# gauravchak/two_tower_models

Measured on AMD Instinct MI355X. Metric: user-item pairs/sec (in-batch softmax train step: fwd + zero_grad + bwd + dense-exact Adam), higher is better.
Workload: dtype f32

## Files before the change

### include/tt_hotpath.h

```cpp
#ifndef TT_HOTPATH_H
#define TT_HOTPATH_H

#include <stdint.h>

#ifdef __cplusplus
extern "C" {
#endif

#define TT_ABI_VERSION 5

#define TT_E_BADARG (-1)
#define TT_E_WORKSPACE (-2)
#define TT_E_UNSUPPORTED (-3)

typedef void* tt_stream_t;

int tt_abi_version(void);
const char* tt_last_error_string(void);

int tt_profile_enable(int on);
int tt_profile_read(const char* kernel, double* total_ms, int64_t* launches);
int tt_profile_filter(const char* kernels);
int tt_profile_pause(int paused);

int tt_gather_rows(const float* table, int64_t n_rows, int64_t dim, const int64_t* ids,
                   int64_t n_ids, float* out, int64_t ld_out, int32_t* oob_flag,
                   tt_stream_t stream);

#define TT_GEMM_NT 0
#define TT_GEMM_NN 1
#define TT_GEMM_TN 2
#define TT_EPI_NONE 0
#define TT_EPI_RELU 1
#define TT_EPI_RELU_MASK 2
int64_t tt_gemm_workspace_bytes(int layout, int64_t M, int64_t N, int64_t K);
int tt_gemm_f32(int layout, int64_t M, int64_t N, int64_t K, const float* A, int64_t lda,
                const float* B, int64_t ldb, float* C, int64_t ldc, const float* bias,
                int epilogue, const float* aux, int64_t ldaux, int accumulate, void* ws,
                int64_t ws_bytes, tt_stream_t stream);
int tt_gemm_tn_colsum_f32(int64_t M, int64_t N, int64_t K, const float* A, int64_t lda, const float* B,
                          int64_t ldb, float* C, int64_t ldc, int accumulate, float* a_colsum, void* ws,
                          int64_t ws_bytes, tt_stream_t stream);
// ... 151 lines not shown
                         const tt_grad_sources* src , int64_t n_ids, const int32_t* sorted_ids,
                         const int32_t* perm, const int32_t* seg_begin, const int32_t* n_unique,
                         void* side, int64_t side_bytes, tt_stream_t stream);

typedef struct {
  const float *W, *M, *V;
  int64_t n_rows, dim;
  const int64_t* ids;
  int64_t n_ids;
  void* side;
  int64_t side_bytes;
} tt_adam_stash_job;
typedef struct {
  float *W, *M, *V;
  int64_t n_rows, dim;
  const tt_grad_sources* src;
  int64_t n_ids;
  const int32_t *sorted_ids, *perm, *seg_begin, *n_unique;
  void* side;
  int64_t side_bytes;
} tt_adam_finish_job;
int tt_adam_begin_ids(double* hyper, float* tab, int64_t tab_steps, const tt_adam_stash_job* jobs, int32_t n_jobs,
                      tt_stream_t stream);
int tt_adam_tables_finish(const tt_adam_finish_job* jobs, int32_t n_jobs, const double* hyper, tt_stream_t stream);
int tt_adam_begin_ids_planes(double* hyper, float* tab, int64_t tab_steps, const tt_adam_stash_job* jobs, int32_t n_jobs,
                             int32_t planes, tt_stream_t stream);

int tt_stream_create_low_priority(void** out_stream);
int tt_stream_destroy(void* stream);

int tt_adam_advance_tab(double* hyper, float* tab, int64_t tab_steps, tt_stream_t stream);
int tt_adam_rows_catchup(float* W, float* M, float* V, int64_t n_rows, int64_t dim, const int64_t* ids,
                         int64_t n_ids, int32_t* last_step, const double* hyper, const float* tab,
                         int64_t tab_steps, tt_stream_t stream);
int tt_adam_table_lazy(float* W, float* M, float* V, int64_t n_rows, int64_t dim, const double* hyper,
                       const tt_grad_sources* src , int64_t n_ids, const int32_t* sorted_ids,
                       const int32_t* perm, const int32_t* seg_begin, const int32_t* n_unique, void* ws,
                       int64_t ws_bytes, int32_t* last_step, const float* tab, int64_t tab_steps,
                       tt_stream_t stream);
int tt_adam_table_flush(float* W, float* M, float* V, int64_t n_rows, int64_t dim, int32_t* last_step,
                        const double* hyper, const float* tab, int64_t tab_steps, tt_stream_t stream);

typedef struct tt_adam_tensor_s {
  float* p;
  const float* g;
  float* m;
  float* v;
  int64_t n;
} tt_adam_tensor;
int tt_adam_dense(const tt_adam_tensor* tensors , int32_t n_tensors, const double* hyper,
                  tt_stream_t stream);
int tt_pack_grads(const tt_adam_tensor* tensors , int32_t n_tensors, tt_stream_t stream);
int tt_copy_buffers(const tt_adam_tensor* buffers , int32_t n_buffers, tt_stream_t stream);
int tt_stream_copy(const void* src, void* dst, int64_t bytes, tt_stream_t stream);
int64_t tt_mfma_probe_flops(int dtype, int32_t iters);
int tt_mfma_probe(int dtype, int32_t iters, float* sink , int64_t sink_floats, tt_stream_t stream);

int tt_hist_embed_pool(const float* table, int64_t n_rows, int64_t dim, const int64_t* ids,
                       int64_t B, int64_t H, const float* pe, float* x, float* pooled,
                       int64_t ld_pooled, int32_t* oob_flag, tt_stream_t stream);
int tt_hist_dx_pool_bwd(const float* dqkv, const float* w_in, int64_t B, int64_t H, int64_t D, const float* d_pooled,
                        int64_t ld_pooled, float* dx, tt_stream_t stream);

int tt_hist_pool_bwd(float* dx, int64_t B, int64_t H, int64_t dim, const float* d_pooled,
                     int64_t ld_pooled, tt_stream_t stream);
int tt_attn_fwd(const float* qkv, int64_t B, int64_t H, int64_t D, int64_t heads, float* ctx,
                float* lse, tt_stream_t stream);
int tt_attn_bwd(const float* qkv, const float* ctx, const float* lse, const float* d_ctx,
                int64_t B, int64_t H, int64_t D, int64_t heads, float* d_qkv, tt_stream_t stream);
int tt_enc_last_supported(int64_t H, int64_t D, int64_t heads);
int tt_enc_last_fwd(const float* x, int64_t B, int64_t H, int64_t D, int64_t heads, const float* w_in,
                    const float* b_in, const float* w_out, const float* b_out, float* recent, int64_t ld_recent,
                    float* q0, float* t, float* probs, float* xbar, float* ctx0, tt_stream_t stream);
int64_t tt_enc_last_bwd_workspace_bytes(int64_t B, int64_t H, int64_t D, int64_t heads);
// ... 109 lines not shown
```

### two_tower_models_amd/_native.py

```python
from __future__ import annotations

import ctypes as C
import os
from typing import Optional

import torch

_PKG = os.path.dirname(os.path.abspath(__file__))
LIB_PATH = os.path.join(_PKG, "lib", "libtt_hotpath.so")

TT_GEMM_NT, TT_GEMM_NN, TT_GEMM_TN = 0, 1, 2
TT_EPI_NONE, TT_EPI_RELU, TT_EPI_RELU_MASK = 0, 1, 2
TT_F32, TT_BF16, TT_F16X2 = 0, 1, 2
TT_E_BADARG, TT_E_WORKSPACE, TT_E_UNSUPPORTED = -1, -2, -3
TT_DEBIAS_COMBINED, TT_DEBIAS_POSITION, TT_DEBIAS_USER = 0, 1, 2
TT_COMM_ID_BYTES = 128
TT_COMM_F32, TT_COMM_I32, TT_COMM_I64, TT_COMM_U8 = 0, 1, 2, 3
TT_COMM_SUM, TT_COMM_MAX = 0, 1
TT_MAX_GRAD_SOURCES = 4
ABI_VERSION = 5

_vp, _i64, _i32, _int = C.c_void_p, C.c_int64, C.c_int32, C.c_int


class GradSources(C.Structure):

    _fields_ = [
        ("rows", _vp * TT_MAX_GRAD_SOURCES),
        ("ld", _i64 * TT_MAX_GRAD_SOURCES),
        ("first", _i64 * (TT_MAX_GRAD_SOURCES + 1)),
        ("n_sources", _i32),
    ]


class AdamTensor(C.Structure):

    _fields_ = [("p", _vp), ("g", _vp), ("m", _vp), ("v", _vp), ("n", _i64)]


class AdamStashJob(C.Structure):

    _fields_ = [("W", _vp), ("M", _vp), ("V", _vp), ("n_rows", _i64), ("dim", _i64), ("ids", _vp), ("n_ids", _i64),
                ("side", _vp), ("side_bytes", _i64)]


class AdamFinishJob(C.Structure):

    _fields_ = [("W", _vp), ("M", _vp), ("V", _vp), ("n_rows", _i64), ("dim", _i64), ("src", C.POINTER(GradSources)),
                ("n_ids", _i64), ("sorted_ids", _vp), ("perm", _vp), ("seg_begin", _vp), ("n_unique", _vp), ("side", _vp),
                ("side_bytes", _i64)]


class TowerFwdSide(C.Structure):
# ... 73 lines not shown
    "tt_inbatch_ce_bwd_kept": (_int, [_vp, _i64, _i64, _i64, _i64, _i64, _vp, _vp, _vp, _i64, _vp, _i64, _vp, _i64, _vp]),
    "tt_ce16_supported": (_int, [_i64, _i64, _i64]),
    "tt_ce16_workspace_bytes": (_i64, [_i64, _i64, _i64]),
    "tt_ce16_fwd_du_keep": (_int, [_vp, _i64, _vp, _i64, _i64, _i64, _i64, _i64, _vp, _vp, _vp, _i64, _vp, _i64, _vp, _i64, _vp]),
    "tt_ce16_bwd_kept": (_int, [_vp, _i64, _i64, _i64, _i64, _i64, _vp, _vp, _vp, _i64, _vp, _i64, _vp, _i64, _vp]),
    "tt_ce16_bwd_recompute": (_int, [_vp, _i64, _vp, _i64, _i64, _i64, _i64, _i64, _vp, _vp, _vp, _i64, _vp, _i64, _int, _vp]),
    "tt_scale_rows": (_int, [_vp, _i64, _vp, _i64, _i64, _vp, _i64, _vp]),
    "tt_weighted_mean_loss": (_int, [_vp, _i64, _i64, _vp, _vp, _vp, _vp, _vp, _vp]),
    "tt_value_weights": (_int, [_vp, _i64, _i64, _vp, _vp, _vp, _vp]),
    "tt_weighted_loss_global": (_int, [_vp, _vp, _vp, _i64, C.c_float, _vp, _vp, _vp]),
    "tt_debias_loss_workspace_bytes": (_i64, [_i64, _i64, _i64]),
    "tt_debias_loss_fwd": (_int, [_int, _vp, _vp, _i64, _i64, _vp, _vp, _i64, _vp, _vp, _i64, _i64, _vp, _vp, _vp, _vp, _i64,
                                  _vp, _vp]),
    "tt_debias_loss_bwd": (_int, [_int, _vp, _vp, _i64, _vp, _i64, _vp, _i64, _i64, _vp, _vp, _i64, _vp, _vp, _i64, _vp, _vp,
                                  _vp, _vp]),
    "tt_rowgrad_workspace_bytes": (_i64, [_i64]),
    "tt_rowgrad_plan": (_int, [_vp, _i64, _i64, _vp, _vp, _vp, _vp, _vp, _vp, _i64, _vp]),
    "tt_rowgrad_dense": (_int, [C.POINTER(GradSources), _i64, _i64, _vp, _vp, _vp, _vp, _vp, _vp]),
    "tt_adam_advance": (_int, [_vp, _vp]),
    "tt_adam_table_workspace_bytes": (_i64, [_i64, _i64]),
    "tt_adam_table": (_int, [_vp, _vp, _vp, _i64, _i64, _vp, C.POINTER(GradSources), _i64, _vp, _vp, _vp,
                             _vp, _vp, _i64, _vp]),
    "tt_adam_table_stash": (_int, [_vp, _vp, _vp, _i64, _i64, _i64, _vp, _vp, _vp, _vp, _vp, _i64, _vp]),
    "tt_adam_table_stash_ids": (_int, [_vp, _vp, _vp, _i64, _i64, _vp, _i64, _vp, _i64, _vp]),
    "tt_adam_table_sweep": (_int, [_vp, _vp, _vp, _i64, _i64, _vp, _vp]),
    "tt_adam_tables_sweep": (_int, [C.POINTER(AdamTensor), _i32, _vp, _i32, _vp]),
    "tt_adam_marks_words": (_i64, [_i64]),
    "tt_adam_marked_supported": (_int, [_i64]),
    "tt_adam_mark_rows": (_int, [_vp, _i64, _i64, _vp, _i64, _vp]),
    "tt_adam_tables_sweep_marked": (_int, [C.POINTER(AdamTensor), C.POINTER(_i64), C.POINTER(_vp), _i32, _vp, _i32, _vp]),
    "tt_adam_table_finish": (_int, [_vp, _vp, _vp, _i64, _i64, _vp, C.POINTER(GradSources), _i64, _vp, _vp, _vp,
                                    _vp, _vp, _i64, _vp]),
    "tt_adam_advance_tab": (_int, [_vp, _vp, _i64, _vp]),
    "tt_adam_rows_catchup": (_int, [_vp, _vp, _vp, _i64, _i64, _vp, _i64, _vp, _vp, _vp, _i64, _vp]),
    "tt_adam_table_lazy": (_int, [_vp, _vp, _vp, _i64, _i64, _vp, C.POINTER(GradSources), _i64, _vp, _vp, _vp, _vp,
                                  _vp, _i64, _vp, _vp, _i64, _vp]),
    "tt_adam_table_flush": (_int, [_vp, _vp, _vp, _i64, _i64, _vp, _vp, _vp, _i64, _vp]),
    "tt_stream_create_low_priority": (_int, [C.POINTER(_vp)]),
    "tt_stream_destroy": (_int, [_vp]),
    "tt_adam_dense": (_int, [C.POINTER(AdamTensor), _i32, _vp, _vp]),
    "tt_pack_grads": (_int, [C.POINTER(AdamTensor), _i32, _vp]),
    "tt_copy_buffers": (_int, [C.POINTER(AdamTensor), _i32, _vp]),
    "tt_hist_embed_pool": (_int, [_vp, _i64, _i64, _vp, _i64, _i64, _vp, _vp, _vp, _i64, _vp, _vp]),
    "tt_hist_dx_pool_bwd": (_int, [_vp, _vp, _i64, _i64, _i64, _vp, _i64, _vp, _vp]),
    "tt_hist_pool_bwd": (_int, [_vp, _i64, _i64, _i64, _vp, _i64, _vp]),
    "tt_attn_fwd": (_int, [_vp, _i64, _i64, _i64, _i64, _vp, _vp, _vp]),
    "tt_attn_bwd": (_int, [_vp, _vp, _vp, _vp, _i64, _i64, _i64, _i64, _vp, _vp]),
    "tt_enc_last_supported": (_int, [_i64, _i64, _i64]),
    "tt_enc_last_fwd": (_int, [_vp, _i64, _i64, _i64, _i64, _vp, _vp, _vp, _vp, _vp, _i64, _vp, _vp, _vp, _vp, _vp, _vp]),
    "tt_enc_last_bwd_workspace_bytes": (_i64, [_i64, _i64, _i64, _i64]),
    "tt_enc_last_bwd": (_int, [_vp, _i64, _i64, _i64, _i64, _vp, _vp, _vp, _i64, _vp, _vp, _vp, _vp, _vp, _vp, _vp, _vp,
                               _vp, _vp, _vp, _i64, _vp]),
    "tt_enc_last_bwd_data": (_int, [_vp, _i64, _i64, _i64, _i64, _vp, _vp, _vp, _i64, _vp, _vp, _vp, _vp, _i64, _vp]),
    "tt_enc_last_bwd_weights": (_int, [_vp, _i64, _i64, _i64, _i64, _vp, _i64, _vp, _vp, _vp, _vp, _vp, _vp, _vp, _vp, _i64, _vp]),
    "tt_stream_copy": (_int, [_vp, _vp, _i64, _vp]),
    "tt_mfma_probe_flops": (_i64, [_int, _i32]),
    "tt_mfma_probe": (_int, [_int, _i32, _vp, _i64, _vp]),
    "tt_rowgrad_plan_jobs_supported": (_int, [_i64]),
    "tt_rowgrad_plan_jobs": (_int, [C.POINTER(PlanJob), _i32, _vp, _vp]),
    "tt_route_workspace_bytes": (_i64, [_i64, _i32]),
    "tt_route_count": (_int, [_vp, _i64, _i64, _i64, _i32, _vp, _vp, _vp, _vp, _i64, _vp]),
    "tt_route_build": (_int, [_vp, _i64, _i64, _i64, _i32, _i64, _vp, _i64, _vp, _vp, _vp, _vp, _vp]),
    "tt_route_localize": (_int, [_vp, _i64, _i64, _i64, _vp, _vp]),
    "tt_route_count_jobs": (_int, [C.POINTER(RouteJob), _i32, _i32, _vp, _vp]),
    "tt_route_build_jobs": (_int, [C.POINTER(RouteJob), _i32, _i32, _vp, _vp]),
    "tt_route_serve_jobs": (_int, [C.POINTER(RouteServeJob), _i32, _vp]),
    "tt_comm_unique_id": (_int, [_vp]),
    "tt_comm_init": (_int, [_vp, _i32, _i32, C.POINTER(_vp)]),
    "tt_comm_destroy": (_int, [_vp]),
    "tt_comm_size": (_int, [_vp, C.POINTER(_i32), C.POINTER(_i32)]),
# ... 182 lines not shown
```

### two_tower_models_amd/csrc/adam.hip

```cpp
#include <stdlib.h>

#include "common.hpp"

namespace tt {

constexpr int SWEEP_MAX_TABLES_DECL = 4;

constexpr int SWEEP_DEFAULT_PERSIST = 3;

struct AdamConst {
  float one_minus_b1, b2, one_minus_b2, eps, neg_step_size, inv_bc2_sqrt;
};

__device__ __forceinline__ AdamConst load_hyper(const double* __restrict__ h) {
  AdamConst c;
  c.one_minus_b1 = (float)(1.0 - h[1]);
  c.b2 = (float)h[2];
  c.one_minus_b2 = (float)(1.0 - h[2]);
  c.eps = (float)h[3];
  c.neg_step_size = (float)(-h[5]);
  c.inv_bc2_sqrt = (float)(1.0 / h[6]);
  return c;
}

// ... 457 lines not shown
__global__ __launch_bounds__(256) void adam_mark_rows_kernel(const int64_t* __restrict__ ids, int64_t n_ids, int64_t n_rows,
                                                             unsigned* __restrict__ marks) {
  const int64_t i = (int64_t)blockIdx.x * 256 + threadIdx.x;
  if (i >= n_ids) return;
  const int64_t row = ids[i];
  if (row >= 0 && row < n_rows) atomicOr(&marks[row >> 5], 1u << (row & 31));
}

__global__ __launch_bounds__(256) void adam_sweep_scalar_kernel(float* __restrict__ W, float* __restrict__ M,
                                                                float* __restrict__ V, int64_t i0, int64_t n,
                                                                const double* __restrict__ hyper) {
  const AdamConst c = load_hyper(hyper);
  const int64_t stride = (int64_t)gridDim.x * blockDim.x;
  for (int64_t i = i0 + (int64_t)blockIdx.x * blockDim.x + threadIdx.x; i < n; i += stride) {
    float p = W[i], m = M[i], v = V[i];
    adam_elem_zero_grad(p, m, v, c);
    W[i] = p; M[i] = m; V[i] = v;
  }
}

__device__ __forceinline__ void replay_consts(AdamConst& c, const double* __restrict__ h, const float* __restrict__ tab,
                                              int64_t cap, int64_t j) {
  if (j < cap) {
    c.neg_step_size = tab[2 * j];
    c.inv_bc2_sqrt = tab[2 * j + 1];
  } else {
    double h5, h6;
    step_consts_from_doubles(h[0], h[1], h[2], (double)j, h5, h6);
    c.neg_step_size = (float)(-h5);
    c.inv_bc2_sqrt = (float)(1.0 / h6);
  }
}

template <int Q>
__device__ __forceinline__ void replay_row_q(float* __restrict__ W, float* __restrict__ M, float* __restrict__ V,
                                             int64_t row, int64_t dim, int32_t from, int32_t to,
                                             const double* __restrict__ hyper, const float* __restrict__ tab,
                                             int64_t cap, int lane) {
  AdamConst c = load_hyper(hyper);
  for (int64_t d0 = 0; d0 < dim; d0 += 64 * Q) {
    float p[Q], m[Q], v[Q];
    bool live = false;
#pragma unroll
    for (int q = 0; q < Q; ++q) {
      const int64_t d = d0 + lane + 64 * q;
      const int64_t at = row * dim + (d < dim ? d : dim - 1);
      p[q] = W[at]; m[q] = M[at]; v[q] = V[at];
      live = live || (d < dim && (m[q] != 0.f || v[q] != 0.f));
    }
    if (!__any(live)) continue;
    for (int32_t j = from + 1; j <= to; ++j) {
      replay_consts(c, hyper, tab, cap, j);
#pragma unroll
      for (int q = 0; q < Q; ++q) adam_elem_zero_grad(p[q], m[q], v[q], c);
    }
#pragma unroll
    for (int q = 0; q < Q; ++q) {
      const int64_t d = d0 + lane + 64 * q;
      if (d < dim) { W[row * dim + d] = p[q]; M[row * dim + d] = m[q]; V[row * dim + d] = v[q]; }
    }
  }
}
__device__ __forceinline__ void replay_row(float* __restrict__ W, float* __restrict__ M, float* __restrict__ V,
                                           int64_t row, int64_t dim, int32_t from, int32_t to,
                                           const double* __restrict__ hyper, const float* __restrict__ tab,
                                           int64_t cap, int lane) {
  from = __builtin_amdgcn_readfirstlane(from);
  to = __builtin_amdgcn_readfirstlane(to);
  if (dim <= 64) replay_row_q<1>(W, M, V, row, dim, from, to, hyper, tab, cap, lane);
  else if (dim <= 128) replay_row_q<2>(W, M, V, row, dim, from, to, hyper, tab, cap, lane);
  else replay_row_q<4>(W, M, V, row, dim, from, to, hyper, tab, cap, lane);
}

__global__ __launch_bounds__(256) void adam_catchup_ids_kernel(float* __restrict__ W, float* __restrict__ M,
                                                               float* __restrict__ V, int64_t n_rows, int64_t dim,
                                                               const int64_t* __restrict__ ids, int64_t n_ids,
                                                               int32_t* __restrict__ last_step,
                                                               const double* __restrict__ hyper, int offset,
                                                               const float* __restrict__ tab, int64_t cap) {
  const int64_t i = (int64_t)blockIdx.x * 4 + (threadIdx.x >> 6);
  if (i >= n_ids) return;
  const int lane = threadIdx.x & 63;
  const int64_t row = ids[i];
  if (row < 0 || row >= n_rows) return;
  const int32_t target = (int32_t)hyper[4] + offset;
  int32_t prev = 0;
  if (lane == 0) prev = atomicMax(&last_step[row], target);
  prev = __shfl(prev, 0, 64);
  if (prev >= target) return;
  replay_row(W, M, V, row, dim, prev, target, hyper, tab, cap, lane);
}

__global__ __launch_bounds__(256) void adam_catchup_plan_kernel(float* __restrict__ W, float* __restrict__ M,
                                                                float* __restrict__ V, int64_t n_rows, int64_t dim,
                                                                const int32_t* __restrict__ sorted_ids,
                                                                const int32_t* __restrict__ seg_begin,
                                                                const int32_t* __restrict__ n_unique,
                                                                int32_t* __restrict__ last_step,
                                                                const double* __restrict__ hyper, int offset, int mark,
                                                                const float* __restrict__ tab, int64_t cap) {
  const int64_t u = (int64_t)blockIdx.x * 4 + (threadIdx.x >> 6);
  if (u >= *n_unique) return;
  const int lane = threadIdx.x & 63;
  const int64_t row = sorted_ids[seg_begin[u]];
  if (row >= n_rows) return;
  const int32_t target = (int32_t)hyper[4] + offset;
  const int32_t prev = last_step[row];
  if (prev < target) replay_row(W, M, V, row, dim, prev, target, hyper, tab, cap, lane);
  if (lane == 0) last_step[row] = target + mark;
}

__global__ __launch_bounds__(256) void adam_flush_kernel(float* __restrict__ W, float* __restrict__ M,
                                                         float* __restrict__ V, int64_t n_rows, int64_t dim,
                                                         int32_t* __restrict__ last_step,
                                                         const double* __restrict__ hyper,
                                                         const float* __restrict__ tab, int64_t cap) {
  const int lane = threadIdx.x & 63;
  const int32_t target = (int32_t)hyper[4];
  const int64_t stride = (int64_t)gridDim.x * 4;
  for (int64_t row = (int64_t)blockIdx.x * 4 + (threadIdx.x >> 6); row < n_rows; row += stride) {
    const int32_t prev = last_step[row];
    if (prev >= target) continue;
    replay_row(W, M, V, row, dim, prev, target, hyper, tab, cap, lane);
    if (lane == 0) last_step[row] = target;
  }
}

constexpr int ADAM_BATCH = 64;
struct AdamBatch { tt_adam_tensor t[ADAM_BATCH]; };
__global__ __launch_bounds__(256) void adam_dense_kernel(const AdamBatch ts, const double* __restrict__ hyper) {
  const tt_adam_tensor t = ts.t[blockIdx.y];
  const AdamConst c = load_hyper(hyper);
  const int64_t stride = (int64_t)gridDim.x * blockDim.x;
  for (int64_t i = (int64_t)blockIdx.x * blockDim.x + threadIdx.x; i < t.n; i += stride) {
    float p = t.p[i], m = t.m[i], v = t.v[i];
    adam_elem(p, m, v, t.g[i], c);
    t.p[i] = p; t.m[i] = m; t.v[i] = v;
  }
}

__global__ __launch_bounds__(256) void pack_grads_kernel(const AdamBatch ts) {
  const tt_adam_tensor t = ts.t[blockIdx.y];
  const int64_t stride = (int64_t)gridDim.x * blockDim.x;
  for (int64_t i = (int64_t)blockIdx.x * blockDim.x + threadIdx.x; i < t.n; i += stride) t.p[i] = t.g[i];
}

__global__ __launch_bounds__(256) void copy_buffers_kernel(const AdamBatch ts) {
  const tt_adam_tensor t = ts.t[blockIdx.y];
  char* dst = reinterpret_cast<char*>(t.p);
  const char* src = reinterpret_cast<const char*>(t.g);
  const int64_t stride = (int64_t)gridDim.x * blockDim.x, i0 = (int64_t)blockIdx.x * blockDim.x + threadIdx.x;
  const bool vec = ((reinterpret_cast<uintptr_t>(dst) | reinterpret_cast<uintptr_t>(src)) & 15) == 0;
  const int64_t n16 = vec ? t.n / 16 : 0;
  for (int64_t i = i0; i < n16; i += stride) reinterpret_cast<uint4*>(dst)[i] = reinterpret_cast<const uint4*>(src)[i];
  for (int64_t i = n16 * 16 + i0; i < t.n; i += stride) dst[i] = src[i];
}
// ... 337 lines not shown
      if (rc) return rc;
    }
    return 0;
  }
  FinishJobs a{};
  a.n = n_jobs;
  unsigned blocks = 0;
  const int rows_per_block = 256 / lpr;
  for (int i = 0; i < n_jobs; ++i) {
    const tt_adam_finish_job& j = jobs[i];
    a.W[i] = j.W; a.M[i] = j.M; a.V[i] = j.V; a.n_rows[i] = j.n_rows; a.dim[i] = j.dim; a.cap[i] = j.n_ids;
    a.src[i] = *j.src; a.sorted_ids[i] = j.sorted_ids; a.perm[i] = j.perm; a.seg_begin[i] = j.seg_begin; a.n_unique[i] = j.n_unique;
    a.side[i] = reinterpret_cast<const float*>(j.side);
    a.first_block[i] = blocks;
    blocks += (unsigned)ceil_div(j.n_ids, rows_per_block);
  }
  for (int i = n_jobs; i <= SWEEP_MAX_TABLES; ++i) a.first_block[i] = blocks;
  hipStream_t st = S(stream);
  if (lpr == 16) adam_finish_tables_kernel<16><<<blocks, 256, 0, st>>>(a, hyper);
  else if (lpr == 32) adam_finish_tables_kernel<32><<<blocks, 256, 0, st>>>(a, hyper);
  else adam_finish_tables_kernel<64><<<blocks, 256, 0, st>>>(a, hyper);
  return check_launch("adam_finish_tables_kernel");
}

extern "C" int tt_adam_advance_tab(double* hyper, float* tab, int64_t tab_steps, tt_stream_t stream) {
  if (!hyper || !tab) return fail_arg("tt_adam_advance_tab: null pointer");
  if (tab_steps <= 0) return fail_arg("tt_adam_advance_tab: sizes");
  adam_advance_kernel<<<1, 1, 0, S(stream)>>>(hyper, tab, tab_steps);
  return check_launch("adam_advance_kernel");
}

extern "C" int tt_adam_rows_catchup(float* W, float* M, float* V, int64_t n_rows, int64_t dim, const int64_t* ids,
                                    int64_t n_ids, int32_t* last_step, const double* hyper, const float* tab,
                                    int64_t tab_steps, tt_stream_t stream) {
  if (!W || !M || !V || !ids || !last_step || !hyper || !tab) return fail_arg("tt_adam_rows_catchup: null pointer");
  if (n_rows <= 0 || dim <= 0 || n_ids <= 0) return fail_arg("tt_adam_rows_catchup: sizes");
  adam_catchup_ids_kernel<<<(unsigned)ceil_div(n_ids, 4), 256, 0, S(stream)>>>(W, M, V, n_rows, dim, ids, n_ids, last_step, hyper, 0, tab, tab_steps);
  return check_launch("adam_catchup_ids_kernel");
}

extern "C" int tt_adam_table_lazy(float* W, float* M, float* V, int64_t n_rows, int64_t dim, const double* hyper,
                                  const tt_grad_sources* src, int64_t n_ids, const int32_t* sorted_ids,
                                  const int32_t* perm, const int32_t* seg_begin, const int32_t* n_unique,
                                  void* ws, int64_t ws_bytes, int32_t* last_step, const float* tab,
                                  int64_t tab_steps, tt_stream_t stream) {
  if (!W || !M || !V || !hyper || !sorted_ids || !perm || !seg_begin || !n_unique || !ws || !last_step || !tab)
    return fail_arg("tt_adam_table_lazy: null pointer");
  if (n_rows <= 0 || dim <= 0 || n_ids <= 0) return fail_arg("tt_adam_table_lazy: sizes");
  if (!check_sources(src, n_ids, dim)) return fail_arg("tt_adam_table_lazy: gradient sources");
  if (ws_bytes < tt_adam_table_workspace_bytes(n_ids, dim)) { set_error("tt_adam_table_lazy: workspace"); return TT_E_WORKSPACE; }
  hipStream_t st = S(stream);
  const unsigned blocks = (unsigned)ceil_div(n_ids, 4);
  adam_catchup_plan_kernel<<<blocks, 256, 0, st>>>(W, M, V, n_rows, dim, sorted_ids, seg_begin, n_unique, last_step, hyper, -1, 1, tab, tab_steps);
  int rc = check_launch("adam_catchup_plan_kernel");
  if (rc) return rc;
  adam_touched_kernel<false><<<blocks, 256, 0, st>>>(W, M, V, n_rows, dim, hyper, *src, sorted_ids, perm, seg_begin, n_unique, reinterpret_cast<float*>(ws), n_ids);
  if ((rc = check_launch("adam_touched_kernel"))) return rc;
  adam_writeback_kernel<<<blocks, 256, 0, st>>>(W, M, V, n_rows, dim, sorted_ids, seg_begin, perm, n_unique, reinterpret_cast<const float*>(ws), n_ids);
  return check_launch("adam_writeback_kernel");
}

extern "C" int tt_adam_table_flush(float* W, float* M, float* V, int64_t n_rows, int64_t dim, int32_t* last_step,
                                   const double* hyper, const float* tab, int64_t tab_steps, tt_stream_t stream) {
  if (!W || !M || !V || !last_step || !hyper || !tab) return fail_arg("tt_adam_table_flush: null pointer");
  if (n_rows <= 0 || dim <= 0) return fail_arg("tt_adam_table_flush: sizes");
  const int64_t want = ceil_div(n_rows, 4);
  const int64_t cap = (int64_t)device_cu_count() * 32;
  ProfScope prof("adam_flush_kernel", S(stream));
  adam_flush_kernel<<<(unsigned)(want < cap ? want : cap), 256, 0, S(stream)>>>(W, M, V, n_rows, dim, last_step, hyper, tab, tab_steps);
  return check_launch("adam_flush_kernel");
}

extern "C" int tt_adam_dense(const tt_adam_tensor* tensors, int32_t n_tensors, const double* hyper,
                             tt_stream_t stream) {
  if (!tensors || !hyper) return fail_arg("tt_adam_dense: null pointer");
  if (n_tensors <= 0) return fail_arg("tt_adam_dense: sizes");
  for (int32_t base = 0; base < n_tensors; base += ADAM_BATCH) {
    const int32_t cnt = (n_tensors - base < ADAM_BATCH) ? n_tensors - base : ADAM_BATCH;
    AdamBatch b;
    int64_t max_n = 1;
    for (int32_t i = 0; i < cnt; ++i) {
      b.t[i] = tensors[base + i];
      if (!b.t[i].p || !b.t[i].g || !b.t[i].m || !b.t[i].v || b.t[i].n < 0) return fail_arg("tt_adam_dense: descriptor");
      if (b.t[i].n > max_n) max_n = b.t[i].n;
    }
    const int64_t bx = ceil_div(max_n, 1024) < 1024 ? ceil_div(max_n, 1024) : 1024;
    adam_dense_kernel<<<dim3((unsigned)bx, (unsigned)cnt), 256, 0, S(stream)>>>(b, hyper);
    const int rc = check_launch("adam_dense_kernel");
    if (rc) return rc;
  }
  return 0;
}

extern "C" int tt_pack_grads(const tt_adam_tensor* tensors, int32_t n_tensors, tt_stream_t stream) {
  if (!tensors) return fail_arg("tt_pack_grads: null pointer");
  if (n_tensors <= 0) return fail_arg("tt_pack_grads: sizes");
  for (int32_t base = 0; base < n_tensors; base += ADAM_BATCH) {
    const int32_t cnt = (n_tensors - base < ADAM_BATCH) ? n_tensors - base : ADAM_BATCH;
    AdamBatch b;
    int64_t max_n = 1;
    for (int32_t i = 0; i < cnt; ++i) {
      b.t[i] = tensors[base + i];
// ... 70 lines not shown
```

### two_tower_models_amd/optim.py

```python
from __future__ import annotations

import ctypes as C
import os
import sys
import weakref
from typing import Dict, Iterable, List, Optional, Sequence

import torch

from . import _native as N
from . import ops


_RELEASE_AT_LOGITS = True
_SPLIT_MIN_IDS = 65536
_MARK_ROWS = True
_HOLD_SWEEP = True


class _TableStep:

    __slots__ = ("plan", "side", "announced", "marked", "n_rows")

    def __init__(self, plan, side, announced=False, marked=False, n_rows=0):
# ... 20 lines not shown
                 eps: float = 1e-8, overlap_sweep=True, lazy: bool = False) -> None:
        if lr < 0 or eps < 0 or not (0 <= betas[0] < 1) or not (0 <= betas[1] < 1):
            raise ValueError("invalid Adam hyper-parameters")
        super().__init__(params, dict(lr=lr, betas=betas, eps=eps))
        if len(self.param_groups) != 1:
            raise ValueError("DenseExactAdam supports a single parameter group")
        self._params: List[torch.nn.Parameter] = [p for p in self.param_groups[0]["params"]]
        self._tables = [p for p in self._params if getattr(p, "_tt_is_table", False)]
        self._dense = [p for p in self._params if not getattr(p, "_tt_is_table", False)]
        for p in self._tables:
            p._tt_rowgrads = []
            p._tt_lookups = []
            p._tt_active = None
            p._tt_optimizer = weakref.ref(self)
        if overlap_sweep not in (True, False, "forward"):
            raise ValueError('overlap_sweep must be True, False or "forward"')
        self._sharded = [p for p in self._tables if getattr(p, "_tt_shard", None) is not None]
        if self._sharded:
            if len(self._sharded) != len(self._tables):
                raise ValueError("either every embedding table of the model is row-sharded or none is")
            if lazy:
                raise ValueError("the deferred (lazy) schedule is a single-GPU schedule; row-sharded tables use the dense-exact sweep")
            overlap_sweep = "forward"
        self._flat_g: Optional[torch.Tensor] = None
        self.lazy = bool(lazy)
        self.overlap_sweep = False if self.lazy else overlap_sweep
        self._last_step: Dict[int, torch.Tensor] = {}
        self._tab: Optional[torch.Tensor] = None
        self._tab_steps = 0
        self._host_steps = 0
        self._resume_step = 0
        self._prefetch_done: Optional[torch.cuda.Event] = None
        self._prefetch_keep = None
        if self.lazy:
            for p in self._tables:
                p._tt_lazy = _LazyRows(self, p)
        self._hyper = None
        self._ready = False
        self._side_stream: Optional[torch.cuda.Stream] = None
        self.capture_overlap = False
        self._sweep_wgs = 0
        self._tune = None
        self._tune_done: List[list] = []
        self._tune_state = None
        self._plan_stream: Optional[torch.cuda.Stream] = None
        self._plan_done: Optional[torch.cuda.Event] = None
        self._plans_pending = False
        self._plan_ready: Optional[torch.cuda.Event] = None
        self._begun: Optional[Dict[torch.nn.Parameter, _TableStep]] = None
        self._sweep_done: Optional[torch.cuda.Event] = None
        self._side_bufs: Dict[int, torch.Tensor] = {}
        self._marks: Dict[int, torch.Tensor] = {}
        self._sweep_pending = None
        self._sweep_pending_marked = False
        self._sweep_events = None
        self._catchup_last: Dict[int, tuple] = {}

    def _init_state(self) -> None:
        dev = N.require_device(*self._params)
        g = self.param_groups[0]
        self._hyper = torch.tensor([g["lr"], g["betas"][0], g["betas"][1], g["eps"], 0.0, 0.0, 0.0, 0.0],
                                   dtype=torch.float64, device=dev)
        arena = bool(self._tables) and all(p.is_cuda for p in self._tables) and os.environ.get("TT_ADAM_NO_ARENA") is None
        in_arena = {id(p) for p in self._tables} if arena else set()
        for p in self._params:
            if p.dtype != torch.float32 or not p.is_contiguous():
# ... 75 lines not shown
        if rates:
            torch.cuda.empty_cache()
        self.arena_note = {"candidates_GBps": [round(r, 1) for r in rates], "kept": best, "bytes": nbytes}
        with torch.no_grad():
            for p, (home, m, v) in zip(self._tables, views(arena)):
                st = self.state[p]
                home.copy_(p.data)
                p.data = home
                for key, t in (("exp_avg", m), ("exp_avg_sq", v)):
                    if key in st:
                        t.copy_(st[key])
                    else:
                        t.zero_()
                    st[key] = t
        self._arena = arena

    def _catch_up(self, p: torch.nn.Parameter, ids: torch.Tensor) -> None:
        if not self._ready or self._host_steps == 0 or not p.is_cuda or ids.numel() == 0:
            return
        cur = torch.cuda.current_stream()
        if self._prefetch_done is not None:
            cur.wait_event(self._prefetch_done)
        if ops._aux_forks[0]:
            prev = self._catchup_last.get(id(p))
            if prev is not None and prev[1] != cur:
                cur.wait_event(prev[0])
        ids = ids.reshape(-1)
        if ids.dtype != torch.int64 or not ids.is_contiguous():
            ids = ids.to(torch.int64).contiguous()
        st = self.state[p]
        N.check(N.load().tt_adam_rows_catchup(p.data_ptr(), st["exp_avg"].data_ptr(), st["exp_avg_sq"].data_ptr(),
                                              p.shape[0], p.shape[1], ids.data_ptr(), ids.numel(),
                                              self._last_step[id(p)].data_ptr(), self._hyper.data_ptr(),
                                              self._tab.data_ptr(), self._tab_steps, N.stream()),
                "tt_adam_rows_catchup")
        if ops._aux_forks[0]:
            ev = torch.cuda.Event()
            ev.record(cur)
            self._catchup_last[id(p)] = (ev, cur)

    @torch.no_grad()
    def prefetch_rows(self, lookups: Dict[torch.nn.Parameter, Sequence[torch.Tensor]]) -> None:
        if not self.lazy or not self._ready or self._host_steps == 0:
            return
        mine = {id(p): p for p in self._tables}
        main = torch.cuda.current_stream()
        ready = torch.cuda.Event()
        ready.record(main)
        self._side_stream.wait_event(ready)
        lib = N.load()
        keep = []
        for p, blocks in lookups.items():
            if id(p) not in mine or not p.is_cuda:
                continue
            st = self.state[p]
            for ids in blocks:
                ids = ids.reshape(-1)
                if ids.dtype != torch.int64 or not ids.is_contiguous():
                    ids = ids.to(torch.int64).contiguous()
                if ids.numel() == 0:
                    continue
                keep.append(ids)
                N.check(lib.tt_adam_rows_catchup(p.data_ptr(), st["exp_avg"].data_ptr(), st["exp_avg_sq"].data_ptr(),
                                                 p.shape[0], p.shape[1], ids.data_ptr(), ids.numel(),
                                                 self._last_step[id(p)].data_ptr(), self._hyper.data_ptr(),
                                                 self._tab.data_ptr(), self._tab_steps,
                                                 self._side_stream.cuda_stream), "tt_adam_rows_catchup")
        self._prefetch_done = torch.cuda.Event()
        self._prefetch_done.record(self._side_stream)
        self._prefetch_keep = keep

    @torch.no_grad()
    def flush(self) -> None:
        if not self.lazy or not self._ready or self._host_steps == 0:
            return
        if self._prefetch_done is not None:
            torch.cuda.current_stream().wait_event(self._prefetch_done)
            self._prefetch_done, self._prefetch_keep = None, None
        lib = N.load()
        for p in self._tables:
            st = self.state[p]
            N.check(lib.tt_adam_table_flush(p.data_ptr(), st["exp_avg"].data_ptr(), st["exp_avg_sq"].data_ptr(),
                                            p.shape[0], p.shape[1], self._last_step[id(p)].data_ptr(),
                                            self._hyper.data_ptr(), self._tab.data_ptr(), self._tab_steps,
                                            N.stream()), "tt_adam_table_flush")

    def state_dict(self):
        self.flush()
        sd = super().state_dict()
        step = torch.tensor(float(self.step_count))
        for st in sd["state"].values():
            st["step"] = step.clone()
        return sd

    def load_state_dict(self, state_dict) -> None:
        super().load_state_dict(state_dict)
        steps = {int(float(st["step"])) for st in self.state.values() if "step" in st}
        if len(steps) > 1:
            raise ValueError("DenseExactAdam needs one common step count for all parameters")
        self._resume_step = steps.pop() if steps else 0
        self._begun = None
        self._ready = False

    def _advance_lazy(self) -> None:
        if self._host_steps + 2 >= self._tab_steps:
            bigger = torch.zeros(4 * self._tab_steps, dtype=torch.float32, device=self._tab.device)
            bigger[: 2 * self._tab_steps].copy_(self._tab)
            self._tab, self._tab_steps = bigger, 2 * self._tab_steps
        N.check(N.load().tt_adam_advance_tab(self._hyper.data_ptr(), self._tab.data_ptr(), self._tab_steps,
                                             N.stream()), "tt_adam_advance_tab")
        self._host_steps += 1

    @property
    def step_count(self) -> int:
        if not self._ready:
            return int(self._resume_step)
        return int(self._hyper[4].item())

# ... 422 lines not shown
                end = torch.cuda.Event(enable_timing=True)
                end.record()
                self._tune[3] = end
                if len(self._tune_done) < 1024:
                    self._tune_done.append(self._tune)
                self._tune = None
        elif self.lazy:
            if self._prefetch_done is not None:
                torch.cuda.current_stream().wait_event(self._prefetch_done)
                self._prefetch_done, self._prefetch_keep = None, None
            self._catchup_last.clear()
            self._advance_lazy()
            todo = []
            for p in self._tables:
                blocks = p._tt_rowgrads
                if p.grad is not None:
                    raise RuntimeError("embedding table received a dense gradient while in row-gradient mode")
                if not blocks:
                    continue
                if all(b.index is not None for b in blocks):
                    blocks = sorted(blocks, key=lambda b: b.index)
                todo.append((p, blocks, ops.RowPlan([b.ids for b in blocks], p.shape[0], slot=f"plan{len(todo)}", defer=True)))
            ops.RowPlan.build_many([plan for _, _, plan in todo])
            for p, blocks, plan in todo:
                plan.attach([b.rows for b in blocks])
                st = self.state[p]
                n_rows, dim = p.shape
                wsp, wsn = ops._ws(p.device, lib.tt_adam_table_workspace_bytes(plan.n, dim), "adam_side")
                N.check(lib.tt_adam_table_lazy(p.data_ptr(), st["exp_avg"].data_ptr(), st["exp_avg_sq"].data_ptr(),
                                               n_rows, dim, hyper, C.byref(plan.sources), plan.n,
                                               plan.sorted_ids.data_ptr(), plan.perm.data_ptr(),
                                               plan.seg_begin.data_ptr(), plan.n_unique.data_ptr(), wsp, wsn,
                                               self._last_step[id(p)].data_ptr(), self._tab.data_ptr(),
                                               self._tab_steps, N.stream()), "tt_adam_table_lazy")
        else:
            N.check(lib.tt_adam_advance(hyper, N.stream()), "tt_adam_advance")
            self._host_steps += 1
            for p in self._tables:
                blocks = p._tt_rowgrads
                st = self.state[p]
                n_rows, dim = p.shape
                if p.grad is not None:
                    raise RuntimeError("embedding table received a dense gradient while in row-gradient mode")
                if blocks:
                    if all(b.index is not None for b in blocks):
                        blocks = sorted(blocks, key=lambda b: b.index)
                    plan = ops.RowPlan.from_grads(blocks, n_rows)
                    wsp, wsn = ops._ws(p.device, lib.tt_adam_table_workspace_bytes(plan.n, dim), "adam_side")
                    N.check(lib.tt_adam_table(p.data_ptr(), st["exp_avg"].data_ptr(), st["exp_avg_sq"].data_ptr(),
                                              n_rows, dim, hyper, C.byref(plan.sources), plan.n,
                                              plan.sorted_ids.data_ptr(), plan.perm.data_ptr(),
                                              plan.seg_begin.data_ptr(), plan.n_unique.data_ptr(), wsp, wsn,
                                              N.stream()), "tt_adam_table")
        for p in self._tables:
            for b in p._tt_rowgrads:
                b.rows
            p._tt_lookups.clear()
            p._tt_rowgrads.clear()
            p._tt_active = None

        if reduce is not None:
            self._finish_dense_allreduce(reduce, lib, hyper)
            return None
        live = [p for p in self._dense if p.grad is not None]
        if live:
            descs = (N.AdamTensor * len(live))()
            keep = []
# ... 10 lines not shown
```

Baseline: 1.524 million.

## Add frozen-row early exit and float2 packed math to lazy Adam replay

The lazy Adam catch-up replay now runs zero-grad steps in blocks of 16. After each block it checks, wave-wide, whether every parameter has become frozen, meaning the update is too small relative to |p| to change it. Once frozen, it advances only m and v, and stops updating m once it reaches a fixed point. The math is done on packed float2 vectors, and the dim>128 Q=4 path is dropped in favour of Q=2 looping. An environment flag restores the plain per-element replay. This is meant to cut the cost of replaying many skipped steps for rarely touched embedding rows, but it depends on a bit-exactness argument about when p stops changing.

```diff
diff --git a/include/tt_hotpath.h b/include/tt_hotpath.h
--- a/include/tt_hotpath.h
+++ b/include/tt_hotpath.h
@@ -7,7 +7,7 @@
 extern "C" {
 #endif
 
-#define TT_ABI_VERSION 5
+#define TT_ABI_VERSION 6
 
 #define TT_E_BADARG (-1)
 #define TT_E_WORKSPACE (-2)
@@ -225,14 +225,15 @@
 int tt_adam_advance_tab(double* hyper, float* tab, int64_t tab_steps, tt_stream_t stream);
 int tt_adam_rows_catchup(float* W, float* M, float* V, int64_t n_rows, int64_t dim, const int64_t* ids,
                          int64_t n_ids, int32_t* last_step, const double* hyper, const float* tab,
-                         int64_t tab_steps, tt_stream_t stream);
+                         int64_t tab_steps, int32_t replay_plain, tt_stream_t stream);
 int tt_adam_table_lazy(float* W, float* M, float* V, int64_t n_rows, int64_t dim, const double* hyper,
                        const tt_grad_sources* src , int64_t n_ids, const int32_t* sorted_ids,
                        const int32_t* perm, const int32_t* seg_begin, const int32_t* n_unique, void* ws,
                        int64_t ws_bytes, int32_t* last_step, const float* tab, int64_t tab_steps,
-                       tt_stream_t stream);
+                       int32_t replay_plain, tt_stream_t stream);
 int tt_adam_table_flush(float* W, float* M, float* V, int64_t n_rows, int64_t dim, int32_t* last_step,
-                        const double* hyper, const float* tab, int64_t tab_steps, tt_stream_t stream);
+                        const double* hyper, const float* tab, int64_t tab_steps, int32_t replay_plain,
+                        tt_stream_t stream);
 
 typedef struct tt_adam_tensor_s {
   float* p;
diff --git a/two_tower_models_amd/_native.py b/two_tower_models_amd/_native.py
--- a/two_tower_models_amd/_native.py
+++ b/two_tower_models_amd/_native.py
@@ -18,7 +18,7 @@
 TT_COMM_F32, TT_COMM_I32, TT_COMM_I64, TT_COMM_U8 = 0, 1, 2, 3
 TT_COMM_SUM, TT_COMM_MAX = 0, 1
 TT_MAX_GRAD_SOURCES = 4
-ABI_VERSION = 5
+ABI_VERSION = 6
 
 _vp, _i64, _i32, _int = C.c_void_p, C.c_int64, C.c_int32, C.c_int
 
@@ -158,10 +158,10 @@
     "tt_adam_table_finish": (_int, [_vp, _vp, _vp, _i64, _i64, _vp, C.POINTER(GradSources), _i64, _vp, _vp, _vp,
                                     _vp, _vp, _i64, _vp]),
     "tt_adam_advance_tab": (_int, [_vp, _vp, _i64, _vp]),
-    "tt_adam_rows_catchup": (_int, [_vp, _vp, _vp, _i64, _i64, _vp, _i64, _vp, _vp, _vp, _i64, _vp]),
+    "tt_adam_rows_catchup": (_int, [_vp, _vp, _vp, _i64, _i64, _vp, _i64, _vp, _vp, _vp, _i64, _i32, _vp]),
     "tt_adam_table_lazy": (_int, [_vp, _vp, _vp, _i64, _i64, _vp, C.POINTER(GradSources), _i64, _vp, _vp, _vp, _vp,
-                                  _vp, _i64, _vp, _vp, _i64, _vp]),
-    "tt_adam_table_flush": (_int, [_vp, _vp, _vp, _i64, _i64, _vp, _vp, _vp, _i64, _vp]),
+                                  _vp, _i64, _vp, _vp, _i64, _i32, _vp]),
+    "tt_adam_table_flush": (_int, [_vp, _vp, _vp, _i64, _i64, _vp, _vp, _vp, _i64, _i32, _vp]),
     "tt_stream_create_low_priority": (_int, [C.POINTER(_vp)]),
     "tt_stream_destroy": (_int, [_vp]),
     "tt_adam_dense": (_int, [C.POINTER(AdamTensor), _i32, _vp, _vp]),
diff --git a/two_tower_models_amd/csrc/adam.hip b/two_tower_models_amd/csrc/adam.hip
--- a/two_tower_models_amd/csrc/adam.hip
+++ b/two_tower_models_amd/csrc/adam.hip
@@ -513,44 +513,139 @@
   }
 }
 
+typedef float float2v __attribute__((ext_vector_type(2)));
+constexpr int REPLAY_BLOCK = 16;
+
+__device__ __forceinline__ void adam_pair_zero_grad(float2v& p, float2v& m, float2v& v, const AdamConst& c) {
+  m = __builtin_elementwise_fma((float2v)(c.one_minus_b1), -m, m);
+  v = v * (float2v)(c.b2);
+  float2v s;
+  s.x = __builtin_amdgcn_sqrtf(v.x); s.y = __builtin_amdgcn_sqrtf(v.y);
+  float2v den = __builtin_elementwise_fma(s, (float2v)(c.inv_bc2_sqrt), (float2v)(c.eps));
+  float2v r;
+  r.x = __builtin_amdgcn_rcpf(fmaxf(den.x, 1e-30f)); r.y = __builtin_amdgcn_rcpf(fmaxf(den.y, 1e-30f));
+  const float2v ratio = m * r;
+  p = __builtin_elementwise_fma((float2v)(c.neg_step_size), ratio, p);
+}
+__device__ __forceinline__ bool replay_frozen_elem(float p, float m, float v, float K) {
+  const float ap = fabsf(p);
+  return fabsf(m) * K <= ap && ap >= 1.17549435e-38f && ap < __builtin_inff() && v >= 0.f && v < __builtin_inff();
+}
+
+template <int Q> struct ReplayVec { using type = float2v; static constexpr int n = Q / 2; };
+template <> struct ReplayVec<1> { using type = float; static constexpr int n = 1; };
+__device__ __forceinline__ float get_elem(float x, int) { return x; }
+__device__ __forceinline__ float get_elem(float2v x, int i) { return i ? x.y : x.x; }
+__device__ __forceinline__ void set_elem(float& x, int, float a) { x = a; }
+__device__ __forceinline__ void set_elem(float2v& x, int i, float a) { if (i) x.y = a; else x.x = a; }
+__device__ __forceinline__ void replay_step(float& p, float& m, float& v, const AdamConst& c, bool) {
+  adam_elem_zero_grad(p, m, v, c);
+}
+__device__ __forceinline__ void replay_step(float2v& p, float2v& m, float2v& v, const AdamConst& c, bool plain) {
+  if (plain) {
+    float a = p.x, b = m.x, d = v.x, e = p.y, f = m.y, g = v.y;
+    adam_elem_zero_grad(a, b, d, c);
+    adam_elem_zero_grad(e, f, g, c);
+    p.x = a; m.x = b; v.x = d; p.y = e; m.y = f; v.y = g;
+  } else {
+    adam_pair_zero_grad(p, m, v, c);
+  }
+}
+__device__ __forceinline__ float replay_m_step(float m, const AdamConst& c) { return fmaf(c.one_minus_b1, -m, m); }
+__device__ __forceinline__ float2v replay_m_step(float2v m, const AdamConst& c) {
+  return __builtin_elementwise_fma((float2v)(c.one_minus_b1), -m, m);
+}
+__device__ __forceinline__ bool same_bits(float a, float b) { return __float_as_uint(a) == __float_as_uint(b); }
+__device__ __forceinline__ bool same_bits(float2v a, float2v b) { return same_bits(a.x, b.x) && same_bits(a.y, b.y); }
+
 template <int Q>
 __device__ __forceinline__ void replay_row_q(float* __restrict__ W, float* __restrict__ M, float* __restrict__ V,
                                              int64_t row, int64_t dim, int32_t from, int32_t to,
                                              const double* __restrict__ hyper, const float* __restrict__ tab,
-                                             int64_t cap, int lane) {
+                                             int64_t cap, int lane, int plain) {
+  using T = typename ReplayVec<Q>::type;
+  constexpr int NV = ReplayVec<Q>::n;
+  constexpr int PER = Q / NV;
   AdamConst c = load_hyper(hyper);
+  const bool hyper_ok = !plain && hyper[1] >= 0.0 && hyper[1] <= 0.9999 && hyper[2] >= 0.0 && hyper[2] < 1.0 &&
+                        c.eps >= 1e-30f && c.eps <= 1.0f;
+  const float k_eps = hyper_ok ? 134217728.0f / c.eps : 0.f;
   for (int64_t d0 = 0; d0 < dim; d0 += 64 * Q) {
-    float p[Q], m[Q], v[Q];
+    T p[NV], m[NV], v[NV];
     bool live = false;
 #pragma unroll
     for (int q = 0; q < Q; ++q) {
       const int64_t d = d0 + lane + 64 * q;
       const int64_t at = row * dim + (d < dim ? d : dim - 1);
-      p[q] = W[at]; m[q] = M[at]; v[q] = V[at];
-      live = live || (d < dim && (m[q] != 0.f || v[q] != 0.f));
+      const float mq = M[at], vq = V[at];
+      set_elem(p[q / PER], q % PER, W[at]); set_elem(m[q / PER], q % PER, mq); set_elem(v[q / PER], q % PER, vq);
+      live = live || (d < dim && (mq != 0.f || vq != 0.f));
     }
     if (!__any(live)) continue;
-    for (int32_t j = from + 1; j <= to; ++j) {
-      replay_consts(c, hyper, tab, cap, j);
-#pragma unroll
-      for (int q = 0; q < Q; ++q) adam_elem_zero_grad(p[q], m[q], v[q], c);
+    int32_t j = from + 1;
+    bool frozen = false;
+    while (j <= to) {
+      const int32_t end = (plain || to - j < REPLAY_BLOCK) ? to : j + REPLAY_BLOCK - 1;
+      for (; j <= end; ++j) {
+        replay_consts(c, hyper, tab, cap, j);
+#pragma unroll
+        for (int q = 0; q < NV; ++q) replay_step(p[q], m[q], v[q], c, plain);
+      }
+      if (hyper_ok && j <= to) {
+        const float s_abs = fabsf(c.neg_step_size);
+        const float K = k_eps * s_abs;
+        bool ok = s_abs >= 7.888609e-31f;
+#pragma unroll
+        for (int q = 0; q < Q; ++q)
+          ok = ok && replay_frozen_elem(get_elem(p[q / PER], q % PER), get_elem(m[q / PER], q % PER), get_elem(v[q / PER], q % PER), K);
+        if (__all(ok)) { frozen = true; break; }
+      }
+    }
+    if (frozen) {
+      int32_t left = to - j + 1;
+      while (left > 0) {
+        bool stopped = true;
+#pragma unroll
+        for (int q = 0; q < NV; ++q) stopped = stopped && same_bits(replay_m_step(m[q], c), m[q]);
+        if (__all(stopped)) break;
+        if (left >= REPLAY_BLOCK) {
+#pragma unroll
+          for (int i = 0; i < REPLAY_BLOCK; ++i) {
+#pragma unroll
+            for (int q = 0; q < NV; ++q) { m[q] = replay_m_step(m[q], c); v[q] = v[q] * c.b2; }
+          }
+          left -= REPLAY_BLOCK;
+        } else {
+          for (; left > 0; --left) {
+#pragma unroll
+            for (int q = 0; q < NV; ++q) { m[q] = replay_m_step(m[q], c); v[q] = v[q] * c.b2; }
+          }
+        }
+      }
+#pragma unroll 8
+      for (int32_t i = 0; i < left; ++i) {
+#pragma unroll
+        for (int q = 0; q < NV; ++q) v[q] = v[q] * c.b2;
+      }
     }
 #pragma unroll
     for (int q = 0; q < Q; ++q) {
       const int64_t d = d0 + lane + 64 * q;
-      if (d < dim) { W[row * dim + d] = p[q]; M[row * dim + d] = m[q]; V[row * dim + d] = v[q]; }
+      if (d < dim) {
+        W[row * dim + d] = get_elem(p[q / PER], q % PER); M[row * dim + d] = get_elem(m[q / PER], q % PER);
+        V[row * dim + d] = get_elem(v[q / PER], q % PER);
+      }
     }
   }
 }
 __device__ __forceinline__ void replay_row(float* __restrict__ W, float* __restrict__ M, float* __restrict__ V,
                                            int64_t row, int64_t dim, int32_t from, int32_t to,
                                            const double* __restrict__ hyper, const float* __restrict__ tab,
-                                           int64_t cap, int lane) {
+                                           int64_t cap, int lane, int plain) {
   from = __builtin_amdgcn_readfirstlane(from);
   to = __builtin_amdgcn_readfirstlane(to);
-  if (dim <= 64) replay_row_q<1>(W, M, V, row, dim, from, to, hyper, tab, cap, lane);
-  else if (dim <= 128) replay_row_q<2>(W, M, V, row, dim, from, to, hyper, tab, cap, lane);
-  else replay_row_q<4>(W, M, V, row, dim, from, to, hyper, tab, cap, lane);
+  if (dim <= 64) replay_row_q<1>(W, M, V, row, dim, from, to, hyper, tab, cap, lane, plain);
+  else replay_row_q<2>(W, M, V, row, dim, from, to, hyper, tab, cap, lane, plain);
 }
 
 __global__ __launch_bounds__(256) void adam_catchup_ids_kernel(float* __restrict__ W, float* __restrict__ M,
@@ -558,7 +653,7 @@
                                                                const int64_t* __restrict__ ids, int64_t n_ids,
                                                                int32_t* __restrict__ last_step,
                                                                const double* __restrict__ hyper, int offset,
-                                                               const float* __restrict__ tab, int64_t cap) {
+                                                               const float* __restrict__ tab, int64_t cap, int plain) {
   const int64_t i = (int64_t)blockIdx.x * 4 + (threadIdx.x >> 6);
   if (i >= n_ids) return;
   const int lane = threadIdx.x & 63;
@@ -569,7 +664,7 @@
   if (lane == 0) prev = atomicMax(&last_step[row], target);
   prev = __shfl(prev, 0, 64);
   if (prev >= target) return;
-  replay_row(W, M, V, row, dim, prev, target, hyper, tab, cap, lane);
+  replay_row(W, M, V, row, dim, prev, target, hyper, tab, cap, lane, plain);
 }
 
 __global__ __launch_bounds__(256) void adam_catchup_plan_kernel(float* __restrict__ W, float* __restrict__ M,
@@ -579,7 +674,7 @@
                                                                 const int32_t* __restrict__ n_unique,
                                                                 int32_t* __restrict__ last_step,
                                                                 const double* __restrict__ hyper, int offset, int mark,
-                                                                const float* __restrict__ tab, int64_t cap) {
+                                                                const float* __restrict__ tab, int64_t cap, int plain) {
   const int64_t u = (int64_t)blockIdx.x * 4 + (threadIdx.x >> 6);
   if (u >= *n_unique) return;
   const int lane = threadIdx.x & 63;
@@ -587,7 +682,7 @@
   if (row >= n_rows) return;
   const int32_t target = (int32_t)hyper[4] + offset;
   const int32_t prev = last_step[row];
-  if (prev < target) replay_row(W, M, V, row, dim, prev, target, hyper, tab, cap, lane);
+  if (prev < target) replay_row(W, M, V, row, dim, prev, target, hyper, tab, cap, lane, plain);
   if (lane == 0) last_step[row] = target + mark;
 }
 
@@ -595,14 +690,14 @@
                                                          float* __restrict__ V, int64_t n_rows, int64_t dim,
                                                          int32_t* __restrict__ last_step,
                                                          const double* __restrict__ hyper,
-                                                         const float* __restrict__ tab, int64_t cap) {
+                                                         const float* __restrict__ tab, int64_t cap, int plain) {
   const int lane = threadIdx.x & 63;
   const int32_t target = (int32_t)hyper[4];
   const int64_t stride = (int64_t)gridDim.x * 4;
   for (int64_t row = (int64_t)blockIdx.x * 4 + (threadIdx.x >> 6); row < n_rows; row += stride) {
     const int32_t prev = last_step[row];
     if (prev >= target) continue;
-    replay_row(W, M, V, row, dim, prev, target, hyper, tab, cap, lane);
+    replay_row(W, M, V, row, dim, prev, target, hyper, tab, cap, lane, plain);
     if (lane == 0) last_step[row] = target;
   }
 }
@@ -1006,10 +1101,10 @@
 
 extern "C" int tt_adam_rows_catchup(float* W, float* M, float* V, int64_t n_rows, int64_t dim, const int64_t* ids,
                                     int64_t n_ids, int32_t* last_step, const double* hyper, const float* tab,
-                                    int64_t tab_steps, tt_stream_t stream) {
+                                    int64_t tab_steps, int32_t replay_plain, tt_stream_t stream) {
   if (!W || !M || !V || !ids || !last_step || !hyper || !tab) return fail_arg("tt_adam_rows_catchup: null pointer");
   if (n_rows <= 0 || dim <= 0 || n_ids <= 0) return fail_arg("tt_adam_rows_catchup: sizes");
-  adam_catchup_ids_kernel<<<(unsigned)ceil_div(n_ids, 4), 256, 0, S(stream)>>>(W, M, V, n_rows, dim, ids, n_ids, last_step, hyper, 0, tab, tab_steps);
+  adam_catchup_ids_kernel<<<(unsigned)ceil_div(n_ids, 4), 256, 0, S(stream)>>>(W, M, V, n_rows, dim, ids, n_ids, last_step, hyper, 0, tab, tab_steps, replay_plain != 0);
   return check_launch("adam_catchup_ids_kernel");
 }
 
@@ -1017,7 +1112,7 @@
                                   const tt_grad_sources* src, int64_t n_ids, const int32_t* sorted_ids,
                                   const int32_t* perm, const int32_t* seg_begin, const int32_t* n_unique,
                                   void* ws, int64_t ws_bytes, int32_t* last_step, const float* tab,
-                                  int64_t tab_steps, tt_stream_t stream) {
+                                  int64_t tab_steps, int32_t replay_plain, tt_stream_t stream) {
   if (!W || !M || !V || !hyper || !sorted_ids || !perm || !seg_begin || !n_unique || !ws || !last_step || !tab)
     return fail_arg("tt_adam_table_lazy: null pointer");
   if (n_rows <= 0 || dim <= 0 || n_ids <= 0) return fail_arg("tt_adam_table_lazy: sizes");
@@ -1025,7 +1120,7 @@
   if (ws_bytes < tt_adam_table_workspace_bytes(n_ids, dim)) { set_error("tt_adam_table_lazy: workspace"); return TT_E_WORKSPACE; }
   hipStream_t st = S(stream);
   const unsigned blocks = (unsigned)ceil_div(n_ids, 4);
-  adam_catchup_plan_kernel<<<blocks, 256, 0, st>>>(W, M, V, n_rows, dim, sorted_ids, seg_begin, n_unique, last_step, hyper, -1, 1, tab, tab_steps);
+  adam_catchup_plan_kernel<<<blocks, 256, 0, st>>>(W, M, V, n_rows, dim, sorted_ids, seg_begin, n_unique, last_step, hyper, -1, 1, tab, tab_steps, replay_plain != 0);
   int rc = check_launch("adam_catchup_plan_kernel");
   if (rc) return rc;
   adam_touched_kernel<false><<<blocks, 256, 0, st>>>(W, M, V, n_rows, dim, hyper, *src, sorted_ids, perm, seg_begin, n_unique, reinterpret_cast<float*>(ws), n_ids);
@@ -1035,13 +1130,14 @@
 }
 
 extern "C" int tt_adam_table_flush(float* W, float* M, float* V, int64_t n_rows, int64_t dim, int32_t* last_step,
-                                   const double* hyper, const float* tab, int64_t tab_steps, tt_stream_t stream) {
+                                   const double* hyper, const float* tab, int64_t tab_steps, int32_t replay_plain,
+                                   tt_stream_t stream) {
   if (!W || !M || !V || !last_step || !hyper || !tab) return fail_arg("tt_adam_table_flush: null pointer");
   if (n_rows <= 0 || dim <= 0) return fail_arg("tt_adam_table_flush: sizes");
   const int64_t want = ceil_div(n_rows, 4);
   const int64_t cap = (int64_t)device_cu_count() * 32;
   ProfScope prof("adam_flush_kernel", S(stream));
-  adam_flush_kernel<<<(unsigned)(want < cap ? want : cap), 256, 0, S(stream)>>>(W, M, V, n_rows, dim, last_step, hyper, tab, tab_steps);
+  adam_flush_kernel<<<(unsigned)(want < cap ? want : cap), 256, 0, S(stream)>>>(W, M, V, n_rows, dim, last_step, hyper, tab, tab_steps, replay_plain != 0);
   return check_launch("adam_flush_kernel");
 }
 
diff --git a/two_tower_models_amd/optim.py b/two_tower_models_amd/optim.py
--- a/two_tower_models_amd/optim.py
+++ b/two_tower_models_amd/optim.py
@@ -76,6 +76,7 @@
         self._resume_step = 0
         self._prefetch_done: Optional[torch.cuda.Event] = None
         self._prefetch_keep = None
+        self._replay_plain = 1 if os.environ.get("TT_ADAM_REPLAY_PLAIN") else 0
         if self.lazy:
             for p in self._tables:
                 p._tt_lazy = _LazyRows(self, p)
@@ -217,7 +218,7 @@
         N.check(N.load().tt_adam_rows_catchup(p.data_ptr(), st["exp_avg"].data_ptr(), st["exp_avg_sq"].data_ptr(),
                                               p.shape[0], p.shape[1], ids.data_ptr(), ids.numel(),
                                               self._last_step[id(p)].data_ptr(), self._hyper.data_ptr(),
-                                              self._tab.data_ptr(), self._tab_steps, N.stream()),
+                                              self._tab.data_ptr(), self._tab_steps, self._replay_plain, N.stream()),
                 "tt_adam_rows_catchup")
         if ops._aux_forks[0]:
             ev = torch.cuda.Event()
@@ -249,7 +250,7 @@
                 N.check(lib.tt_adam_rows_catchup(p.data_ptr(), st["exp_avg"].data_ptr(), st["exp_avg_sq"].data_ptr(),
                                                  p.shape[0], p.shape[1], ids.data_ptr(), ids.numel(),
                                                  self._last_step[id(p)].data_ptr(), self._hyper.data_ptr(),
-                                                 self._tab.data_ptr(), self._tab_steps,
+                                                 self._tab.data_ptr(), self._tab_steps, self._replay_plain,
                                                  self._side_stream.cuda_stream), "tt_adam_rows_catchup")
         self._prefetch_done = torch.cuda.Event()
         self._prefetch_done.record(self._side_stream)
@@ -268,7 +269,7 @@
             N.check(lib.tt_adam_table_flush(p.data_ptr(), st["exp_avg"].data_ptr(), st["exp_avg_sq"].data_ptr(),
                                             p.shape[0], p.shape[1], self._last_step[id(p)].data_ptr(),
                                             self._hyper.data_ptr(), self._tab.data_ptr(), self._tab_steps,
-                                            N.stream()), "tt_adam_table_flush")
+                                            self._replay_plain, N.stream()), "tt_adam_table_flush")
 
     def state_dict(self):
         self.flush()
@@ -757,7 +758,7 @@
                                                plan.sorted_ids.data_ptr(), plan.perm.data_ptr(),
                                                plan.seg_begin.data_ptr(), plan.n_unique.data_ptr(), wsp, wsn,
                                                self._last_step[id(p)].data_ptr(), self._tab.data_ptr(),
-                                               self._tab_steps, N.stream()), "tt_adam_table_lazy")
+                                               self._tab_steps, self._replay_plain, N.stream()), "tt_adam_table_lazy")
         else:
             N.check(lib.tt_adam_advance(hyper, N.stream()), "tt_adam_advance")
             self._host_steps += 1
```

Result: no change. 1.525 million, median of 5 (+0.0%).
